# sanowl/CUDA-NT-Xent-MPI-NCCL-SimCLR

Hardware: AMD Instinct MI355X
Metric: NT-Xent fwd+bwd samples/sec, B=4096 d=2048, at 1/2/4/8 MI355X (higher is better)
Workload: dtype bf16

## Files before the change

cuda-nt-xent-mpi-nccl-simclr_amd/csrc/include/ntxent/ntxent.h:

```cpp
#pragma once

#include <hip/hip_runtime.h>

#include <cstdint>
#include <stdexcept>
#include <string>
#include <utility>
#include <vector>

namespace ntxent {

constexpr int kWaveSize = 64;
constexpr int kTile = 256;
constexpr int kTileElems = kTile * kTile;
constexpr int kKStepBytes = 128;
constexpr int kGemmThreads = 512;
constexpr int kLdsPerCU = 160 * 1024;
constexpr int kNumXcd = 8;

enum class DType : int { F32 = 0, F16 = 1, BF16 = 2, FP8 = 3 };

inline size_t dtype_size(DType t) { return t == DType::F32 ? 4 : (t == DType::FP8 ? 1 : 2); }
inline const char* dtype_name(DType t) {
  return t == DType::F32 ? "fp32" : (t == DType::F16 ? "fp16" : (t == DType::BF16 ? "bf16" : "fp8"));
// ... 130 lines not shown
void launch_lse(const float2* part, const float* ypos, float* lse2_all, float* cpos,
                float* block_loss, float* loss_sum, const Geometry& g, hipStream_t stream,
                DType tr_dtype = DType::F16, const void* zq = nullptr, void* zqt = nullptr,
                const Q8Stats* q8 = nullptr, const RawRows* raw = nullptr, bool fold_order = false);

int dot_slots(const Geometry& g);
void launch_coef(DType comp, const void* sbuf, void* cbuf, const float* lse2_all, const float* cpos,
                 const int4* tiles, int ntiles, const Geometry& g, hipStream_t stream,
                 void* mbuf = nullptr, float* dotp = nullptr, const Q8Stats* q8 = nullptr, bool half_c = false);
void launch_dot_reduce(const float* dotp, float* dot, const Geometry& g, hipStream_t stream);

void launch_coef_gemm(DType comp, const void* zq_local, const void* zq_all, void* cbuf,
                      const float* lse2_all, const float* cpos, const int4* tiles, int ntiles,
                      const GemmWorkspace& ws, const Geometry& g, hipStream_t stream,
                      const BlockView& bv = BlockView{}, float* dotp = nullptr);

struct NormFuse {
  const void* h = nullptr;
  DType in = DType::BF16;
  const float* inv = nullptr;
  const float* dot = nullptr;
  const float* grad_out = nullptr;
  void* dh = nullptr;
  const float* dotp = nullptr;
  int* dot_cnt = nullptr;
};
bool launch_dz(DType comp, const void* cbuf, const void* zqt_all, const int4* tiles, int ntiles,
               void* dz, const GemmWorkspace& ws, const Geometry& g, hipStream_t stream, bool out_f16 = false,
               const NormFuse* nf = nullptr, const Q8Stats* q8 = nullptr, const float* cpos = nullptr,
               bool half_c = false);
bool dz_half_c_eligible(DType comp, const Geometry& g, int n_dz, const GemmWorkspace& ws);
void set_half_c(bool on);
bool half_c_enabled();
bool dz_dot_fold_eligible(DType comp, const Geometry& g, int n_dz, const GemmWorkspace& ws);
void set_dot_fold(bool on);
bool dot_fold_enabled();
void set_dot_fold_spin(int polls);
int dot_fold_spin();

void launch_dz_view(DType comp, const void* a, long long a_panel_tiles, const void* b, long long b_kblk_cols,
                    long long b_kblk_stride, int k_tiles, const int4* tiles, int ntiles, void* out, bool accum,
                    const GemmWorkspace& ws, const Geometry& g, hipStream_t stream, bool out_f16 = false);

void launch_norm_bwd(DType in, const float* slabs, int nslabs, const void* h,
                     const float* inv, const float* grad_out, void* dh, const Geometry& g,
                     hipStream_t stream, const void* xslabs = nullptr, int nx = 0, float* dot_out = nullptr);

void launch_tau_grad(const float* dot, const float* grad_out, float* dtau, const Geometry& g, hipStream_t stream,
                     double* share64 = nullptr);

constexpr int kSmallMaxRows = 2048;
constexpr int kSmallMaxDk = 256;
bool small_path_eligible(const Geometry& g, DType comp);
int small_bwd_splits(const Geometry& g);
int small_rows_pad(const Geometry& g);
size_t small_scratch_bytes(const Geometry& g, int splits);
constexpr int kSmallFuseMaxRows = 1024;
bool small_fwd_fused(const Geometry& g);
void set_small_fuse_rows(int rows);
int small_fuse_rows_override();
void launch_small_fwd(DType in, DType comp, const void* h, void* zq, float* inv, float* ypos, float* lse2,
                      float* arow, float* loss, void* scratch, const Geometry& g, hipStream_t stream);
void launch_small_bwd(DType in, DType comp, const void* zq, const void* h, const float* inv, const float* lse2,
                      const float* arow, const float* grad_out, void* dh, void* scratch, const Geometry& g,
                      hipStream_t stream, int splits = 0, float* dot_out = nullptr);

// ... 56 lines not shown
```

cuda-nt-xent-mpi-nccl-simclr_amd/csrc/kernels/ntxent_kernels.hip:

```cpp

#include "../include/ntxent/ntxent.h"
#include "device_common.h"
#include "host_common.h"
#include "sim_gemm.h"

#include <atomic>
#include <algorithm>
#include <cmath>
#include <cstdio>
#include <cstdlib>
#include <mutex>
#include <string>
#include <type_traits>
#include <vector>
#include <unordered_map>

namespace ntxent {
namespace dev {

template <typename T> __device__ __forceinline__ void load8(const T* p, float (&v)[8]);
template <> __device__ __forceinline__ void load8<float>(const float* p, float (&v)[8]) {
  const f32x4 a = *reinterpret_cast<const f32x4*>(p), b = *reinterpret_cast<const f32x4*>(p + 4);
  v[0] = a[0]; v[1] = a[1]; v[2] = a[2]; v[3] = a[3]; v[4] = b[0]; v[5] = b[1]; v[6] = b[2]; v[7] = b[3];
}
// ... 722 lines not shown
  __syncthreads();
  if (threadIdx.x < 32 && blockIdx.x * 32 + (int)threadIdx.x < rows) {
    float t = 0.f;
#pragma unroll
    for (int g = 0; g < 8; ++g) t += part[g][threadIdx.x];
    dot[blockIdx.x * 32 + threadIdx.x] = t;
  }
}

constexpr int kTauGradThreads = 1024;
__global__ __launch_bounds__(kTauGradThreads) void tau_grad_kernel(const float* __restrict__ dot, int rows,
                                                                   const float* __restrict__ grad_out, double scale,
                                                                   float* __restrict__ dtau,
                                                                   double* __restrict__ share64) {
  __shared__ double part[kTauGradThreads];
  double t = 0.0;
  for (int i = threadIdx.x; i < rows; i += kTauGradThreads) t += (double)dot[i];
  part[threadIdx.x] = t;
  __syncthreads();
#pragma unroll
  for (int n = kTauGradThreads / 2; n > 0; n >>= 1) {
    if ((int)threadIdx.x < n) part[threadIdx.x] += part[threadIdx.x + n];
    __syncthreads();
  }
  if (threadIdx.x == 0) {
    const double v = (double)grad_out[0] * scale * part[0];
    if (dtau) dtau[0] = (float)v;
    else share64[0] = v;
  }
}

}

namespace {
void set_operand_scales(dev::SimParams& p, DType comp, const Geometry& g) {
  p.acc_scale = p.y_scale;
  p.scale_off = comp == DType::FP8 ? g.dim_k8 : 0;
}

#if NTXENT_TIMING
struct TimingBuf {
  unsigned long long* buf = nullptr;
  size_t cap = 0, n = 0;
  unsigned long long* prepare(int grid, hipStream_t stream) {
    n = (size_t)grid * dev::kTimingItems * dev::kTimingMarks;
    if (n > cap) {
      if (buf) NTXENT_HIP_CHECK(hipFree(buf));
      NTXENT_HIP_CHECK(hipMalloc(&buf, n * 8));
      cap = n;
    }
    NTXENT_HIP_CHECK(hipMemsetAsync(buf, 0, n * 8, stream));
    return buf;
  }
  void dump(const std::string& name, int grid, hipStream_t stream) const {
    const char* dir = std::getenv("NTXENT_TIMING_OUT");
    if (!dir) return;
    std::vector<unsigned long long> h(n);
    NTXENT_HIP_CHECK(hipStreamSynchronize(stream));
    NTXENT_HIP_CHECK(hipMemcpy(h.data(), buf, n * 8, hipMemcpyDeviceToHost));
    const std::string f = std::string(dir) + "/" + name + "_g" + std::to_string(grid) + ".bin";
    if (FILE* fp = std::fopen(f.c_str(), "wb")) {
      const int hdr[3] = {grid, dev::kTimingItems, dev::kTimingMarks};
      std::fwrite(hdr, sizeof(int), 3, fp);
      std::fwrite(h.data(), 8, n, fp);
      std::fclose(fp);
    }
  }
};
#endif

template <typename Tc, int MODE>
void launch_sim_gemm(int grid, const dev::SimParams& p_in, hipStream_t stream) {
#if NTXENT_TIMING
  static TimingBuf tb;
  dev::SimParams p = p_in;
  p.tstamp = tb.prepare(grid, stream);
#else
  const dev::SimParams& p = p_in;
#endif
  if (MODE == dev::kModeFwd && !p.fixed_shift)
    hipLaunchKernelGGL((dev::sim_gemm_kernel<Tc, MODE, MODE == dev::kModeFwd ? 0 : 1>), dim3(grid), dim3(kGemmThreads), 0,
                       stream, p);
  else
    hipLaunchKernelGGL((dev::sim_gemm_kernel<Tc, MODE>), dim3(grid), dim3(kGemmThreads), 0, stream, p);
#if NTXENT_TIMING
  tb.dump("gemm_m" + std::to_string(MODE) + "_e" + std::to_string(sizeof(Tc)), grid, stream);
#endif
}

dev::SimParams base_params(const Geometry& g) {
  dev::SimParams p{};
  p.R = g.rows;
  p.Rpad = g.rows_pad;
  p.n_half = g.rows / 2;
  p.own0 = g.rank * g.rows_pad;
  p.row_tile0 = g.rank * g.row_tiles;
  p.col_tiles = g.col_tiles;
  p.b_tile0 = 0;
  p.c_ld = g.col_tiles;
  p.c_tile0 = 0;
  p.y_scale = g.inv_temp * dev::kLog2e;
  p.acc_scale = p.y_scale;
  p.fixed_shift = (2.0f * p.y_scale < 120.0f) ? 1 : 0;
  return p;
}

constexpr int kDiagTickets = 14;
size_t sk_counter_bytes(int num_cus) {
  return ((size_t)std::max(2, kDiagTickets) * std::max(1, num_cus) * 4 + 255) / 256 * 256;
}

int apply_schedule(dev::SimParams& p, int ntiles, const GemmWorkspace& ws, hipStream_t stream) {
// ... 280 lines not shown
  });
  NTXENT_HIP_CHECK(hipGetLastError());
}

static std::atomic<bool> g_small_path{true};
static std::atomic<int> g_small_splits{0};
static std::atomic<int> g_small_fuse_rows{-1};
static std::atomic<bool> g_fp8_bwd{true};
static std::atomic<bool> g_raw_fwd{true};
void set_small_path(bool on) { g_small_path = on; }
bool small_path_enabled() { return g_small_path.load(); }
void set_small_splits(int n) { g_small_splits = std::max(0, n); }
int small_splits_override() { return g_small_splits.load(); }
void set_small_fuse_rows(int rows) { g_small_fuse_rows = rows < 0 ? -1 : rows; }
int small_fuse_rows_override() { return g_small_fuse_rows.load(); }
void set_fp8_backward(bool on) { g_fp8_bwd = on; }
void set_raw_forward(bool on) { g_raw_fwd = on; }

static std::atomic<bool> g_lse_fold{[] {
  const char* e = std::getenv("NTXENT_LSE_FOLD");
  return e == nullptr || std::string(e) != "0";
}()};
void set_lse_fold(bool on) { g_lse_fold = on; }

bool lse_fold_enabled() { return g_lse_fold.load(); }
static double lse_loss_fx(const Geometry& g, int nb);

static std::atomic<bool> g_half_c{[] {
  const char* e = std::getenv("NTXENT_HALF_C");
  return e == nullptr || std::string(e) != "0";
}()};
void set_half_c(bool on) { g_half_c = on; }
bool half_c_enabled() { return g_half_c.load(); }

bool dz_half_c_eligible(DType comp, const Geometry& g, int n_dz, const GemmWorkspace& ws) {
  if ((comp != DType::F16 && comp != DType::BF16) || g.world != 1 || n_dz <= 0) return false;
  if ((long long)g.row_tiles * g.col_tiles * kTileElems * 2 >= (1ll << 31)) return false;
  const int cus = ws.sched_cus > 0 ? std::min(ws.sched_cus, ws.num_cus) : ws.num_cus;
  const int nk = (int)((long long)g.rows_pad * 2 / kKStepBytes);
  int pieces = fwd_splitk_pieces(n_dz, nk, cus, 1);
  if (pieces < 3) pieces = 0;
  if (pieces > 0) return ((nk + pieces - 1) / pieces) % 2 == 0;
  return make_schedule(n_dz, nk, cus).sk_tiles == 0;
}
static std::atomic<bool> g_dot_fold{[] {
  const char* e = std::getenv("NTXENT_DOT_FOLD");
  return e == nullptr || std::string(e) != "0";
}()};
void set_dot_fold(bool on) { g_dot_fold = on; }
bool dot_fold_enabled() { return g_dot_fold.load(); }
static std::atomic<int> g_dot_spin{1 << 14};
void set_dot_fold_spin(int polls) { g_dot_spin = polls < 0 ? 0 : polls; }
int dot_fold_spin() { return g_dot_spin.load(); }
bool dz_dot_fold_eligible(DType comp, const Geometry& g, int n_dz, const GemmWorkspace&) {
  return (comp == DType::F16 || comp == DType::BF16) && n_dz > 0 && g.dim % 8 == 0 && dot_fold_enabled();
}
bool raw_forward_enabled() { return g_raw_fwd.load(); }
bool raw_forward_eligible(const Geometry& g, DType in, DType comp) {
  return g.world == 1 && (in == DType::F16 || in == DType::BF16) && (comp == DType::F16 || comp == in) &&
         g.rows % kTile == 0 && g.dim % 64 == 0 && g.dim <= 16384;
}
bool fp8_backward_enabled() { return g_fp8_bwd.load(); }
bool fp8_backward_eligible(const Geometry& g, DType comp) { return comp == DType::FP8 && g.world == 1 && g.dim % 8 == 0; }
int q8_ldt(const Geometry& g) { return (!NTXENT_NO_LDPAD && g.rows_pad % 1024 == 0) ? g.rows_pad + 128 : g.rows_pad; }

#ifndef NTXENT_ZT_SIDE_PER_CU
// ... 506 lines not shown
```

cuda-nt-xent-mpi-nccl-simclr_amd/csrc/kernels/sim_gemm.h:

```cpp
#pragma once

#include "../include/ntxent/ntxent.h"
#include "device_common.h"
#include "pair_mask.h"

#include <type_traits>

namespace ntxent {
namespace dev {

enum SimMode : int { kModeFwd = 0, kModeCoef = 1, kModeDz = 2 };

constexpr int kStageBytes = 2 * kTile * kKStepBytes;
#ifndef NTXENT_GEMM_DMA_AUX
#define NTXENT_GEMM_DMA_AUX 0
#endif
constexpr int kGemmDmaAux = NTXENT_GEMM_DMA_AUX;
#ifndef NTXENT_TIMING
#define NTXENT_TIMING 0
#endif
constexpr int kTimingItems = 8;
constexpr int kTimingMarks = 8;
__device__ __forceinline__ void store16_wt(void* base, long long off, u32x4 v) {
  const unsigned lo = __builtin_amdgcn_readfirstlane((unsigned)off);
  const unsigned hi = __builtin_amdgcn_readfirstlane((unsigned)((unsigned long long)off >> 32));
  const long long f0 = (long long)(((unsigned long long)hi << 32) | lo) - (64ll << 20);
  const long long wb = f0 > 0 ? (f0 & ~0xFFFFFll) : 0;
  const auto rs = __builtin_amdgcn_make_buffer_rsrc(static_cast<char*>(base) + wb, 0, 0x7FFFFFFF, 0x00020000);
  __builtin_amdgcn_raw_buffer_store_b128(v, rs, (int)(off - wb), 0, 16);
}

__device__ __forceinline__ long long ctile_off(int r, int c, int es) { return ((long long)r * kTile + c) * es; }
constexpr int kGemmLds = 2 * kStageBytes;
constexpr int kCtStride = kTile * 2 + 16;
constexpr int kCoefLds = kTile * kCtStride;
constexpr int kCoefWaveLds = 64 * (64 * 2 + 16);
constexpr int kHalfBytes = 128 * kKStepBytes;

struct OperandDesc {
  const char* base;
  long long row_tile_stride;
  long long ld;
  long long kblk;
  long long kblk_stride;
};

struct SimParams {
  OperandDesc A, B;
  const int4* tiles;
  long long kbytes;
  int R, Rpad, n_half, own0, row_tile0, col_tiles;
  int b_tile0;
  int c_ld, c_tile0;
  int c_rot;
  int c_half;
// ... 757 lines not shown
          op[1] = f32x4{o[4], o[5], o[6], o[7]};
        }
      }
      return;
    }
    _Float16* o16 = reinterpret_cast<_Float16*>(out) + ((long long)mt * kTile) * p.ldo + nt * kTile;
#pragma unroll 4
    for (int k = 0; k < 16; ++k) {
      const int idx = tid + kGemmThreads * k, rt = idx >> 5, c = idx & 31;
      const u32x4 v = *(lds_u4*)(lds + rt * 512 + ((c ^ (rt & 15)) << 4));
      *reinterpret_cast<u32x4*>(o16 + (long long)rt * p.ldo + c * 8) = v;
    }
  } else {
#pragma unroll
  for (int mi = 0; mi < 8; ++mi) {
    const long long row = (long long)mt * kTile + rb[mi] + (lane & 15);
#pragma unroll
    for (int ni = 0; ni < 4; ++ni) {
      const int col = nt * kTile + cb[ni] + 4 * (lane >> 4);
      if (p.out_f16) {
        union { _Float16 h[4]; u32x2 u; } pk;
#pragma unroll
        for (int r = 0; r < 4; ++r) pk.h[r] = (_Float16)acc[mi][ni][r];
        *reinterpret_cast<u32x2*>(reinterpret_cast<_Float16*>(out) + row * p.ldo + col) = pk.u;
      } else {
        f32x4* o = reinterpret_cast<f32x4*>(out + row * p.ldo + col);
        *o = p.accum ? *o + acc[mi][ni] : acc[mi][ni];
      }
    }
  }
  }
}

template <typename T, int MODE, int FX = 1>
__global__ __launch_bounds__(kGemmThreads) void sim_gemm_kernel(const SimParams p) {
  typedef typename Mfma<T>::frag frag;
  typedef __attribute__((address_space(3))) const frag lds_frag;
  constexpr int kScaleLds = MODE == kModeCoef ? kCoefLds : kGemmLds;
  constexpr int kFwdRed = kScaleLds + ((std::is_same<T, fp8e4m3>::value || MODE == kModeDz) ? 2048 : 0);
  constexpr int kInvLds = kFwdRed + (MODE == kModeFwd ? 6 * 256 * 8 : 0);
  __shared__ __attribute__((aligned(16))) char smem[kInvLds + (MODE == kModeFwd && !std::is_same<T, fp8e4m3>::value ? 4096 : 0) +
                                                     (MODE == kModeDz && !std::is_same<T, fp8e4m3>::value ? kHPieceExtra : 0)];
  lds_char* lds = (lds_char*)smem;
  typedef __attribute__((address_space(3))) u32x4 lds_u4;

  const int tid = threadIdx.x, lane = tid & 63, w = __builtin_amdgcn_readfirstlane(tid >> 6);
  const int wa = w >> 2, wb = w & 3;
  const int G = gridDim.x;
  const int bid = xcd_remap(blockIdx.x, G);
  const int nk = p.nk;
  KStream sa0, sa1, sb0, sb1;

  unsigned a_vo[2], b_vo[2];
#pragma unroll
  for (int j = 0; j < 2; ++j) {
    const int rl = 8 * j + (lane >> 3);
    const int lchunk = (lane & 7) ^ ((rl >> 1) & 7);
    a_vo[j] = (unsigned)((lane >> 3) * p.A.ld) + lchunk * 16;
    b_vo[j] = (unsigned)((lane >> 3) * p.B.ld) + lchunk * 16;
  }
  constexpr bool kTrCap = MODE == kModeDz && sizeof(T) == 2 && !std::is_same<T, fp8e4m3>::value;
  int tr_end = 0;
  const char* tr_base = nullptr;
  unsigned a_tr_vo = 0, rd_tr = 0;
  if constexpr (kTrCap) {
    const int x = w & 1;
    const int ch = 8 * (((lane >> 3) & 1) ^ x) + 2 * (lane >> 4) + (lane & 1);
// ... 89 lines not shown
        constexpr int sv = decltype(s_c)::value, mv = decltype(mi_c)::value;
        constexpr int off = OFF0 + 8 * sv * 1024 + 256 * mv;
        u32x2 lo, hi;
        asm volatile("ds_read_b64_tr_b16 %0, %2 offset:%c3\n\tds_read_b64_tr_b16 %1, %2 offset:%c4"
                     : "=&v"(lo), "=&v"(hi)
                     : "v"(base), "i"(off), "i"(off + 1024)
                     : "memory");
        af[sv][mv] = __builtin_bit_cast(OP, u32x4{lo[0], lo[1], hi[0], hi[1]});
      };
      typedef std::integral_constant<int, 0> J0;
      typedef std::integral_constant<int, 1> J1;
      typedef std::integral_constant<int, 2> J2;
      typedef std::integral_constant<int, 3> J3;
      one(J0{}, J0{}); one(J0{}, J1{}); one(J0{}, J2{}); one(J0{}, J3{});
      one(J1{}, J0{}); one(J1{}, J1{}); one(J1{}, J2{}); one(J1{}, J3{});
    }
  };
  auto read_b = [&](int buf, int h, OP (&bf)[NS][2]) {
    i32x4 lo[2];
#pragma unroll
    for (int s = 0; s < 2; ++s) {
#pragma unroll
      for (int ni = 0; ni < 2; ++ni) {
        const lds_char* src = lds + rd_b[s] + (buf * kTile + 128 * h + 16 * ni) * kKStepBytes;
        if constexpr (kF8) {
          if (s == 0) lo[ni] = *(lds_i4*)src;
          else bf[0][ni] = __builtin_shufflevector(lo[ni], *(lds_i4*)src, 0, 1, 2, 3, 4, 5, 6, 7);
        } else {
          bf[s][ni] = *(lds_frag*)src;
        }
      }
    }
  };
  auto mma_quadrant = [&](auto qa_c, auto qb_c, OP (&af)[NS][4], OP (&bf)[NS][2]) {
    constexpr int qa = decltype(qa_c)::value, qb = decltype(qb_c)::value;
    __builtin_amdgcn_s_setprio(1);
    if constexpr (kF8) {
      auto mx = [&](auto mi_c, auto ni_c) {
        constexpr int mi = decltype(mi_c)::value, ni = decltype(ni_c)::value;
        f32x4& c = acc[qa * 4 + mi][qb * 2 + ni];
        if constexpr (MODE == kModeDz)
          c = mma_mx_c<qb * 2 + ni, mi>(bf[0][ni], af[0][mi], c, kUnitScale, kUnitScale);
        else
          c = mma_mx_c<mi, qb * 2 + ni>(af[0][mi], bf[0][ni], c, sa_v[qa], sb_v);
        asm volatile("" ::"v"(c));
      };
      typedef std::integral_constant<int, 0> I0;
      typedef std::integral_constant<int, 1> I1;
      typedef std::integral_constant<int, 2> I2;
      typedef std::integral_constant<int, 3> I3;
      mx(I0{}, I0{}); mx(I0{}, I1{}); mx(I1{}, I0{}); mx(I1{}, I1{});
      mx(I2{}, I0{}); mx(I2{}, I1{}); mx(I3{}, I0{}); mx(I3{}, I1{});
    } else {
#pragma unroll
      for (int s = 0; s < 2; ++s)
#pragma unroll
        for (int mi = 0; mi < 4; ++mi)
#pragma unroll
          for (int ni = 0; ni < 2; ++ni) {
            f32x4& c = acc[qa * 4 + mi][qb * 2 + ni];
            c = MODE == kModeDz ? Mfma<T>::mma(bf[s][ni], af[s][mi], c) : Mfma<T>::mma(af[s][mi], bf[s][ni], c);
          }
    }
    __builtin_amdgcn_s_setprio(0);
  };
  const std::integral_constant<int, 0> kI0{};
  const std::integral_constant<int, 1> kI1{};
  auto barrier = [&]() {
    __builtin_amdgcn_s_barrier();
    asm volatile("" ::: "memory");
  };
  auto lds_drain = [&]() { asm volatile("s_waitcnt lgkmcnt(0)" ::: "memory"); };
  auto a0_retire = [&]() { asm volatile("s_waitcnt lgkmcnt(4)" ::: "memory"); };
  constexpr bool kStreamMode = MODE == kModeFwd && !kF8;
  auto dma_wait = [&]() { asm volatile("s_waitcnt vmcnt(8)" ::: "memory"); };
  const int grp = __builtin_amdgcn_readfirstlane(w) >> 2;

  const long long sk_total = (long long)p.sk_tiles * nk;
  const long long it0 = (long long)bid * p.ipb;
  const long long it1 = it0 + p.ipb < sk_total ? it0 + p.ipb : sk_total;
  const int n_dp = p.dp_tiles > bid ? (p.dp_tiles - bid + G - 1) / G : 0;
  long long it = it0;
  auto fetch = [&](int item, int& tile, int& kb, int& ke, int& stile) -> bool {
    stile = -1;
    if (item < n_dp) {
      tile = bid + item * G;
      kb = 0;
      ke = nk;
      return true;
    }
    if (p.splitk) {
      if (item > 0) return false;
      stile = bid % p.sk_tiles;
      kb = (int)((bid / p.sk_tiles) * p.ipb);
      ke = kb + (int)p.ipb < nk ? kb + (int)p.ipb : nk;
      tile = p.dp_tiles + stile;
      return true;
    }
    if (it >= it1) return false;
    stile = (int)(it / nk);
    kb = (int)(it % nk);
    ke = (int)((long long)kb + (it1 - it) < nk ? kb + (it1 - it) : nk);
    it += ke - kb;
    tile = p.dp_tiles + stile;
    return true;
  };
  auto prologue = [&](int tile, int kb, int ke, int slot) {
    const int4 tt = sload_int4(p.tiles, tile);
    if (p.inv_a) stage_inv(tt.x, tt.y, slot);
    if constexpr (kTrCap) {
// ... 3 lines not shown
    const int ns = ke - kb;
    const char* Ab = p.A.base + (long long)tt.x * p.A.row_tile_stride;
    const char* Bb = p.B.base + (long long)(tt.y - p.b_tile0) * p.B.row_tile_stride;
    const long long k0 = (long long)kb * kKStepBytes;
    sa0.init(Ab, k0, p.A, ns); sa1.init(Ab, k0, p.A, ns);
    if constexpr (kTrCap) {
      if (tr_end > kb) {
        sa0.seek(Ab, (long long)tr_end * kKStepBytes, p.A);
        sa1.seek(Ab, (long long)tr_end * kKStepBytes, p.A);
      }
    }
    sb0.init(Bb, k0, p.B, ns); sb1.init(Bb, k0, p.B, ns);
    if constexpr (kF8 && MODE != kModeDz) {
      const int t = threadIdx.x;
      const char* src = (t < 256 ? Ab + (long long)t * p.A.ld : Bb + (long long)(t - 256) * p.B.ld) + p.scale_off;
      __builtin_amdgcn_global_load_lds((const void*)src, (lds_void*)(lds + kScaleLds + 256 * w), 4, 0, 0);
    }
    stage(0, 0, sa0, 0); stage(1, 0, sb0, 0); stage(1, 1, sb1, 0); stage(0, 1, sa1, 0);
    stage(0, 0, sa0, 1); stage(1, 0, sb0, 1); stage(1, 1, sb1, 1);
  };
  const bool streaming = kStreamMode && p.sk_tiles == 0 && nk >= 2 && (nk & 1) == 0;
  bool streamed = false;
  int dstate = 0;
  bool dot_counted = false;
  if constexpr (MODE == kModeDz && !kF8 && sizeof(T) == 2) {
    if (p.dot_nslot > 0) dz_dot_fold(p, lds + kGemmLds, threadIdx.x);
  }
  auto tmark = [&](int item, int k) {
#if NTXENT_TIMING
    if (threadIdx.x == 0 && item < kTimingItems)
      p.tstamp[((long long)blockIdx.x * kTimingItems + item) * kTimingMarks + k] = __builtin_amdgcn_s_memtime();
#endif
  };
  for (int item = 0;; ++item) {
  tmark(item, 0);
  int tile, kb, ke, stile;
  if (streamed) {
    tile = bid + item * G; kb = 0; ke = nk; stile = -1;
  } else {
    if (!fetch(item, tile, kb, ke, stile)) break;
    prologue(tile, kb, ke, item & 1);
  }
  const bool cont = streaming && item + 1 < n_dp;
  const char* na = nullptr;
  const char* nb = nullptr;
  int nmt = 0, nnt = 0;
  if (cont) {
    const int4 tn = sload_int4(p.tiles, bid + (item + 1) * G);
    na = p.A.base + (long long)tn.x * p.A.row_tile_stride;
    nb = p.B.base + (long long)(tn.y - p.b_tile0) * p.B.row_tile_stride;
    nmt = tn.x;
    nnt = tn.y;
  }
  const int4 t = sload_int4(p.tiles, tile);
  const int mt = t.x, nt = t.y;
  const int nsteps = ke - kb;
#pragma unroll
  for (int mi = 0; mi < 8; ++mi)
#pragma unroll
    for (int ni = 0; ni < 4; ++ni) acc[mi][ni] = f32x4{0.f, 0.f, 0.f, 0.f};

  asm volatile("s_waitcnt vmcnt(10)" ::: "memory");
  barrier();
  if constexpr (MODE == kModeDz && !kF8 && sizeof(T) == 2) {
    if (item == 0 && p.dot_cnt != nullptr && threadIdx.x == 0)
      __hip_atomic_fetch_add(p.dot_cnt, 1, __ATOMIC_RELAXED, __HIP_MEMORY_SCOPE_AGENT);
    dot_counted = true;
  }
  if constexpr (kF8 && MODE != kModeDz) {
    const int r16_ = lane & 15;
    unsigned av[8], bv[4];
    lds_get_scales((unsigned)(uintptr_t)(lds + kScaleLds) + 4 * (64 * wa + r16_),
                   (unsigned)(uintptr_t)(lds + kScaleLds) + 4 * (256 + 32 * wb + r16_), av, bv);
    sa_v[0] = pack_low_bytes(av[0], av[1], av[2], av[3]);
    sa_v[1] = pack_low_bytes(av[4], av[5], av[6], av[7]);
    sb_v = pack_low_bytes(bv[0], bv[1], bv[2], bv[3]);
  }
  tmark(item, 1);
  if (grp == 1) barrier();
  bool hpre = false;
  if constexpr (MODE == kModeDz && !kF8)
    hpre = p.ndh != nullptr && (p.nh_dt == 1 || p.nh_dt == 2) && stile < 0 && nsteps == nk && nsteps >= 4 &&
           (nsteps & 1) == 0 && p.R % kTile == 0 && p.nd % kTile == 0;
  auto kstep = [&](const int ks, auto cur_c, auto tail_c, auto tr_c) {
    constexpr int cur = decltype(cur_c)::value, nxt = cur ^ 1;
    constexpr int TAIL = decltype(tail_c)::value;
    constexpr bool TR = decltype(tr_c)::value != 0;
    constexpr int TRM = decltype(tr_c)::value == 0 ? 0 : (decltype(tr_c)::value == 2 ? 1 : 2);
    if constexpr (kStreamMode) {
      if (cont && ks == nsteps - 2) {
        sa0.init(na, 0, p.A, nk); sb0.init(nb, 0, p.B, nk); sb1.init(nb, 0, p.B, nk);
        if (p.inv_a) stage_inv(nmt, nnt, (item + 1) & 1);
      }
      if (cont && ks == nsteps - 1) sa1.init(na, 0, p.A, nk);
    }
    dma_wait(); barrier();
    if constexpr (TR) read_a_tr(cur_c, kI0, af);
    else read_a(cur, 0, af);
    __builtin_amdgcn_sched_barrier(0);
    read_b(cur, 0, bf0);
    if constexpr (TAIL == 2) stage_h(3, mt, nt);
    else stage(0, 1, sa1, nxt, TRM);
    a0_retire(); barrier();
    lds_drain();
    if constexpr (TR) __builtin_amdgcn_sched_barrier(0);
    mma_quadrant(kI0, kI0, af, bf0);
    dma_wait(); barrier();
    read_b(cur, 1, bf1);
    if constexpr (TAIL != 0) stage_h(TAIL == 1 ? 0 : 4, mt, nt);
    else stage(0, 0, sa0, cur, TRM);
    barrier(); lds_drain();
    mma_quadrant(kI0, kI1, af, bf1);
    barrier();
    if constexpr (TR) read_a_tr(cur_c, kI1, af);
    else read_a(cur, 1, af);
    if constexpr (TAIL != 0) stage_h(TAIL == 1 ? 1 : 5, mt, nt);
    else stage(1, 0, sb0, cur);
    barrier(); lds_drain();
    if constexpr (TR) __builtin_amdgcn_sched_barrier(0);
    mma_quadrant(kI1, kI0, af, bf0);
    if constexpr (TAIL != 2) dma_wait();
    barrier();
    if constexpr (TAIL != 0) {
      stage_h(TAIL == 1 ? 2 : 6, mt, nt);
      if constexpr (TAIL == 2) stage_h(7, mt, nt);
    } else {
      stage(1, 1, sb1, cur);
    }
    barrier();
    mma_quadrant(kI1, kI1, af, bf1);
  };
  const std::integral_constant<int, 2> kI2{};
  int ks2 = 0;
  const int nmain = nsteps - (hpre ? 2 : 0);
  if constexpr (kTrCap) {
    const int ntr = tr_end > kb ? (tr_end < ke ? tr_end : ke) - kb : 0;
    for (; ks2 + 3 < ntr; ks2 += 2) {
      kstep(ks2, kI0, kI0, kI1);
      kstep(ks2 + 1, kI1, kI0, kI1);
    }
    if (ks2 + 1 < ntr) {
      kstep(ks2, kI0, kI0, kI2);
      kstep(ks2 + 1, kI1, kI0, kI2);
      ks2 += 2;
    }
  }
  for (; ks2 + 1 < nmain; ks2 += 2) {
    kstep(ks2, kI0, kI0, kI0);
    kstep(ks2 + 1, kI1, kI0, kI0);
  }
  if constexpr (MODE == kModeDz && !kF8) {
    if (hpre) {
      kstep(ks2, kI0, kI1, kI0);
      kstep(ks2 + 1, kI1, kI2, kI0);
      ks2 += 2;
    }
  }
  if (ks2 < nsteps) kstep(ks2, kI0, kI0, kI0);
  if (grp == 0) barrier();
  tmark(item, 2);
  float hiv = 0.f, hdt = 0.f;
  if constexpr (MODE == kModeDz && !kF8) {
    if (hpre && threadIdx.x < kTile) {
      hiv = p.ninv[mt * kTile + threadIdx.x];
      hdt = dz_dot<sizeof(T) == 2>(p, mt * kTile + threadIdx.x, dstate);
    }
  }
  if (kStreamMode && cont) {
    streamed = true;
  } else {
    streamed = false;
    asm volatile("s_waitcnt vmcnt(0)" ::: "memory");
  }
  if constexpr (kStreamMode) {
    lds_drain();
    barrier();
  } else {
    __syncthreads();
  }
  {
  int tid_e = threadIdx.x;
  asm volatile("" : "+v"(tid_e));
  const int tid = tid_e, lane = tid_e & 63, w = tid_e >> 6;
  const int wa = w >> 2, wb = w & 3;
  int rb[8], cb[4];
#pragma unroll
  for (int mi = 0; mi < 8; ++mi) rb[mi] = 128 * (mi >> 2) + 64 * wa + 16 * (mi & 3);
#pragma unroll
  for (int ni = 0; ni < 4; ++ni) cb[ni] = 128 * (ni >> 1) + 32 * wb + 16 * (ni & 1);

  if constexpr (MODE == kModeFwd && !kF8) {
    if (p.inv_a) {
      const unsigned ib = (unsigned)(uintptr_t)(lds + kInvLds) + (unsigned)((item & 1) * 2048);
// ... 836 lines not shown
```

cuda-nt-xent-mpi-nccl-simclr_amd/csrc/runtime/ntxent_torch.cpp:

```cpp
#include <torch/extension.h>
#include <ATen/hip/impl/HIPGuardImplMasqueradingAsCUDA.h>
#include <ATen/hip/impl/HIPStreamMasqueradingAsCUDA.h>
#include <ATen/hip/impl/HIPCachingAllocatorMasqueradingAsCUDA.h>

#include <algorithm>
#include <map>
#include <memory>
#include <atomic>
#include <mutex>
#include <string>
#include <tuple>
#include <vector>

#include "ntxent/engine.h"
#include "ntxent/ntxent.h"
#include "ntxent/step.h"
#include "ntxent/sym_step.h"
#include "../kernels/pair_mask.h"

namespace ntxent {
namespace th {

DType to_dtype(at::ScalarType t) {
  switch (t) {
// ... 1334 lines not shown
  m.def("rccl_unique_id", []() { return py::bytes(ntxent::RcclComm::unique_id()); });
  m.def("get_plan", &get_plan, py::arg("rows"), py::arg("dim"), py::arg("world"), py::arg("rank"),
        py::arg("temperature"), py::arg("compute"), py::arg("device"));
  m.def("choose_compute", [](const std::string& in_dtype, bool mp, const std::string& ov) {
    at::ScalarType t = in_dtype == "float32" ? at::kFloat : (in_dtype == "float16" ? at::kHalf : at::kBFloat16);
    return std::string(ntxent::dtype_name(choose_compute(t, mp, ov)));
  });
  m.def("prep", &prep, py::arg("h"), py::arg("plan"), py::arg("zq_out") = py::none(), py::arg("zq8_out") = py::none());
  m.def("transpose", &transpose, py::arg("zq"), py::arg("plan"), py::arg("zqt_out") = py::none());
  m.def("pos_rank", &pos_rank, py::arg("zq"), py::arg("plan"),
        "Stage op: (rank, pos_cos, hard_neg_cos) of prep's unit rows zq for a world-1 plan.");
  m.def("positive_rank", &positive_rank, py::arg("h"), py::arg("compute") = "auto",
        py::arg("use_mixed_precision") = false,
        "(rank, pos_cos, hard_neg_cos) of stacked views h = [h1; h2] on the current stream: rank[i] counts the "
        "negatives whose cosine is strictly larger than the positive's. compute: auto|fp32|fp16|bf16|fp8, "
        "resolved as for the loss; fp8 computes in fp16.");
  m.def("fwd_stats_range", &fwd_stats_range, py::arg("zq_local"), py::arg("zq_all"), py::arg("plan"), py::arg("part"),
        py::arg("sc"), py::arg("first"), py::arg("count"), py::arg("reserve_cus") = 0);
  m.def("fwd_stats", [](const at::Tensor& zl, const at::Tensor& za, const Plan& P, bool keep) {
    return fwd_stats(zl, za, P, keep, true);
  }, py::arg("zq_local"), py::arg("zq_all"), py::arg("plan"), py::arg("keep_cos"));
  m.def("lse", &lse, py::arg("part"), py::arg("ypos"), py::arg("lse2_all"), py::arg("cpos"), py::arg("plan"),
        py::arg("zq") = py::none(), py::arg("zqt") = py::none());
  m.def("coef", &coef, py::arg("sbuf"), py::arg("lse2_all"), py::arg("cpos"), py::arg("plan"));
  m.def("coef_gemm", &coef_gemm);
  m.def("dz", &dz);
  m.def("set_fp8_backward", &ntxent::set_fp8_backward, py::arg("on"));
  m.def("set_raw_forward", &ntxent::set_raw_forward, py::arg("on"));
  m.def("raw_forward_enabled", &ntxent::raw_forward_enabled);
  m.def("set_lse_fold", &ntxent::set_lse_fold, py::arg("on"));
  m.def("lse_fold_enabled", &ntxent::lse_fold_enabled);
  m.def("set_half_c", &ntxent::set_half_c, py::arg("on"));
  m.def("half_c_enabled", &ntxent::half_c_enabled);
  m.def("set_dot_fold", &ntxent::set_dot_fold, py::arg("on"));
  m.def("dot_fold_enabled", &ntxent::dot_fold_enabled);
  m.def("set_dot_fold_spin", &ntxent::set_dot_fold_spin, py::arg("polls"));
  m.def("dot_fold_spin", &ntxent::dot_fold_spin);
  m.def("fp8_backward_enabled", &ntxent::fp8_backward_enabled);
  m.def("fwd_splitk_pieces", &ntxent::fwd_splitk_pieces, py::arg("ntiles"), py::arg("nk"), py::arg("cus"),
        py::arg("diag_tail"));
  m.def("fwd_diag_remainder", &ntxent::fwd_diag_remainder, py::arg("ntiles"), py::arg("nk"), py::arg("cus"),
        py::arg("diag_tail"), py::arg("f8") = false);
  m.def("norm_bwd", &norm_bwd, py::arg("slabs"), py::arg("h"), py::arg("inv"), py::arg("grad_out"), py::arg("plan"));
  m.def("fwd_stats_tiles", &fwd_stats_tiles, py::arg("zq_local"), py::arg("zq_chunk"), py::arg("b_tile0"),
        py::arg("tiles"), py::arg("plan"), py::arg("part"), py::arg("reserve_cus") = 0);
  m.def("coef_gemm_tiles", &coef_gemm_tiles, py::arg("zq_local"), py::arg("zq_chunk"), py::arg("b_tile0"),
        py::arg("tiles"), py::arg("lse2_all"), py::arg("cpos"), py::arg("plan"), py::arg("c_ld"), py::arg("c_tile0"),
        py::arg("reserve_cus") = 0);
  m.def("dz_block", &dz_block, py::arg("cbuf_block"), py::arg("zqt_chunk"), py::arg("plan"), py::arg("reserve_cus") = 0);
  m.def("dz_view", &dz_view, py::arg("abuf"), py::arg("a_tile0"), py::arg("a_panel_tiles"), py::arg("bbuf"),
        py::arg("b_block0"), py::arg("b_col0"), py::arg("k_tiles"), py::arg("m0"), py::arg("m1"), py::arg("out"),
        py::arg("accum"), py::arg("plan"), py::arg("reserve_cus") = 0);
  {
    const auto plan = py::arg("plan"), bufs = py::arg("bufs");
    const auto reserve = py::arg("reserve_cus") = 0;
    py::class_<SymStep, std::shared_ptr<SymStep>>(m, "SymStep")
        .def_property_readonly("plan", [](const SymStep& S) { return sym_plan_dict(S.sp); })
        .def("prep", sym_phase<>([](const SymStep& S, const Plan& P, SymBundle& x, hipStream_t s) {
          ntxent::sym_prep(S.sp, P.g, x.in, x.b, s);
        }), plan, bufs)
        .def("fwd_tiles_range", sym_phase<int, int, int>([](const SymStep& S, const Plan& P, SymBundle& x, hipStream_t s,
                                                            int first, int count, int reserve_cus) {
          ntxent::sym_fwd_tiles(S.sp, P.g, P.comp, x.b, first, count, gemm_ws(x.like, count, P, reserve_cus), s);
        }), plan, bufs, py::arg("first"), py::arg("count"), reserve)
        .def("lse", sym_phase<>([](const SymStep& S, const Plan& P, SymBundle& x, hipStream_t s) {
          x.b.block_loss = static_cast<float*>(device_scratch(x.like, (size_t)ntxent::lse_scratch_floats(P.g) * 4, 1).data_ptr());
// ... 149 lines not shown
```

Measured before the change: 11.21 million.

## Add two-phase k-step schedule for bf16/fp16 dz GEMM, on by default

Adds a SCHED=2 variant of the similarity GEMM k-step that splits each step into two phases. Each phase reads an A half and both B fragments, then issues two MFMA quadrants back to back, which halves the barriers and DMA waits per step compared with the four-quadrant schedule. The variant is on by default for the dz backward GEMM (fp16/bf16, no split-k) and can be toggled per mode through an env var or Python setters. It also adds finer timing marks and a compile-time switch that disables MFMA for profiling. Holding more fragments live may raise register pressure, and the new vmcnt wait counts must match the DMA issue order.

```diff
diff --git a/cuda-nt-xent-mpi-nccl-simclr_amd/csrc/include/ntxent/ntxent.h b/cuda-nt-xent-mpi-nccl-simclr_amd/csrc/include/ntxent/ntxent.h
--- a/cuda-nt-xent-mpi-nccl-simclr_amd/csrc/include/ntxent/ntxent.h
+++ b/cuda-nt-xent-mpi-nccl-simclr_amd/csrc/include/ntxent/ntxent.h
@@ -186,6 +186,9 @@
 bool dz_half_c_eligible(DType comp, const Geometry& g, int n_dz, const GemmWorkspace& ws);
 void set_half_c(bool on);
 bool half_c_enabled();
+void set_gemm_two_phase(bool on, int which = -1);
+bool gemm_two_phase_enabled(bool dz);
+long long gemm_two_phase_launches(bool dz);
 bool dz_dot_fold_eligible(DType comp, const Geometry& g, int n_dz, const GemmWorkspace& ws);
 void set_dot_fold(bool on);
 bool dot_fold_enabled();
diff --git a/cuda-nt-xent-mpi-nccl-simclr_amd/csrc/kernels/ntxent_kernels.hip b/cuda-nt-xent-mpi-nccl-simclr_amd/csrc/kernels/ntxent_kernels.hip
--- a/cuda-nt-xent-mpi-nccl-simclr_amd/csrc/kernels/ntxent_kernels.hip
+++ b/cuda-nt-xent-mpi-nccl-simclr_amd/csrc/kernels/ntxent_kernels.hip
@@ -778,6 +778,8 @@
 
 }
 
+static void count_two_phase_launch(bool dz);
+
 namespace {
 void set_operand_scales(dev::SimParams& p, DType comp, const Geometry& g) {
   p.acc_scale = p.y_scale;
@@ -824,6 +826,22 @@
 #else
   const dev::SimParams& p = p_in;
 #endif
+  constexpr bool kTwoCap = !std::is_same<Tc, float>::value && !std::is_same<Tc, dev::fp8e4m3>::value &&
+                           (MODE == dev::kModeFwd || MODE == dev::kModeDz);
+  if constexpr (kTwoCap) {
+    if (gemm_two_phase_enabled(MODE == dev::kModeDz) && p.sk_tiles == 0 && !p.splitk) {
+      count_two_phase_launch(MODE == dev::kModeDz);
+      if (MODE == dev::kModeFwd && !p.fixed_shift)
+        hipLaunchKernelGGL((dev::sim_gemm_kernel<Tc, MODE, MODE == dev::kModeFwd ? 0 : 1, 2>), dim3(grid),
+                           dim3(kGemmThreads), 0, stream, p);
+      else
+        hipLaunchKernelGGL((dev::sim_gemm_kernel<Tc, MODE, 1, 2>), dim3(grid), dim3(kGemmThreads), 0, stream, p);
+#if NTXENT_TIMING
+      tb.dump("gemm_m" + std::to_string(MODE) + "_e" + std::to_string(sizeof(Tc)), grid, stream);
+#endif
+      return;
+    }
+  }
   if (MODE == dev::kModeFwd && !p.fixed_shift)
     hipLaunchKernelGGL((dev::sim_gemm_kernel<Tc, MODE, MODE == dev::kModeFwd ? 0 : 1>), dim3(grid), dim3(kGemmThreads), 0,
                        stream, p);
@@ -1170,6 +1188,24 @@
 }()};
 void set_half_c(bool on) { g_half_c = on; }
 bool half_c_enabled() { return g_half_c.load(); }
+
+static constexpr bool kTwoPhaseDefault[2] = {false, true};
+static std::atomic<bool> g_two_phase[2];
+static const bool g_two_phase_init = [] {
+  const char* e = std::getenv("NTXENT_TWO_PHASE");
+  const std::string v = e ? e : "";
+  g_two_phase[0] = e == nullptr ? kTwoPhaseDefault[0] : (v == "fwd" || (v != "0" && v != "dz"));
+  g_two_phase[1] = e == nullptr ? kTwoPhaseDefault[1] : (v == "dz" || (v != "0" && v != "fwd"));
+  return true;
+}();
+void set_gemm_two_phase(bool on, int which) {
+  if (which != 1) g_two_phase[0] = on;
+  if (which != 0) g_two_phase[1] = on;
+}
+bool gemm_two_phase_enabled(bool dz) { return g_two_phase[dz ? 1 : 0].load(); }
+static std::atomic<long long> g_two_phase_launches[2];
+static void count_two_phase_launch(bool dz) { ++g_two_phase_launches[dz ? 1 : 0]; }
+long long gemm_two_phase_launches(bool dz) { return g_two_phase_launches[dz ? 1 : 0].load(); }
 
 bool dz_half_c_eligible(DType comp, const Geometry& g, int n_dz, const GemmWorkspace& ws) {
   if ((comp != DType::F16 && comp != DType::BF16) || g.world != 1 || n_dz <= 0) return false;
diff --git a/cuda-nt-xent-mpi-nccl-simclr_amd/csrc/kernels/sim_gemm.h b/cuda-nt-xent-mpi-nccl-simclr_amd/csrc/kernels/sim_gemm.h
--- a/cuda-nt-xent-mpi-nccl-simclr_amd/csrc/kernels/sim_gemm.h
+++ b/cuda-nt-xent-mpi-nccl-simclr_amd/csrc/kernels/sim_gemm.h
@@ -20,7 +20,10 @@
 #define NTXENT_TIMING 0
 #endif
 constexpr int kTimingItems = 8;
-constexpr int kTimingMarks = 8;
+constexpr int kTimingMarks = 32;
+#ifndef NTXENT_NO_MFMA
+#define NTXENT_NO_MFMA 0
+#endif
 __device__ __forceinline__ void store16_wt(void* base, long long off, u32x4 v) {
   const unsigned lo = __builtin_amdgcn_readfirstlane((unsigned)off);
   const unsigned hi = __builtin_amdgcn_readfirstlane((unsigned)((unsigned long long)off >> 32));
@@ -844,7 +847,7 @@
   }
 }
 
-template <typename T, int MODE, int FX = 1>
+template <typename T, int MODE, int FX = 1, int SCHED = 4>
 __global__ __launch_bounds__(kGemmThreads) void sim_gemm_kernel(const SimParams p) {
   typedef typename Mfma<T>::frag frag;
   typedef __attribute__((address_space(3))) const frag lds_frag;
@@ -1000,10 +1003,17 @@
       }
     }
   };
-  auto mma_quadrant = [&](auto qa_c, auto qb_c, OP (&af)[NS][4], OP (&bf)[NS][2]) {
+  auto mma_quadrant_raw = [&](auto qa_c, auto qb_c, OP (&af)[NS][4], OP (&bf)[NS][2]) __attribute__((always_inline)) {
     constexpr int qa = decltype(qa_c)::value, qb = decltype(qb_c)::value;
-    __builtin_amdgcn_s_setprio(1);
-    if constexpr (kF8) {
+    if constexpr (NTXENT_NO_MFMA != 0 && !kF8) {
+#pragma unroll
+      for (int s = 0; s < NS; ++s) {
+#pragma unroll
+        for (int mi = 0; mi < 4; ++mi) asm volatile("" ::"v"(af[s][mi]));
+#pragma unroll
+        for (int ni = 0; ni < 2; ++ni) asm volatile("" ::"v"(bf[s][ni]));
+      }
+    } else if constexpr (kF8) {
       auto mx = [&](auto mi_c, auto ni_c) {
         constexpr int mi = decltype(mi_c)::value, ni = decltype(ni_c)::value;
         f32x4& c = acc[qa * 4 + mi][qb * 2 + ni];
@@ -1030,6 +1040,16 @@
             c = MODE == kModeDz ? Mfma<T>::mma(bf[s][ni], af[s][mi], c) : Mfma<T>::mma(af[s][mi], bf[s][ni], c);
           }
     }
+  };
+  auto mma_quadrant = [&](auto qa_c, auto qb_c, OP (&af)[NS][4], OP (&bf)[NS][2]) __attribute__((always_inline)) {
+    __builtin_amdgcn_s_setprio(1);
+    mma_quadrant_raw(qa_c, qb_c, af, bf);
+    __builtin_amdgcn_s_setprio(0);
+  };
+  auto mma_half = [&](auto qa_c, OP (&af)[NS][4], OP (&bf0)[NS][2], OP (&bf1)[NS][2]) __attribute__((always_inline)) {
+    __builtin_amdgcn_s_setprio(1);
+    mma_quadrant_raw(qa_c, std::integral_constant<int, 0>{}, af, bf0);
+    mma_quadrant_raw(qa_c, std::integral_constant<int, 1>{}, af, bf1);
     __builtin_amdgcn_s_setprio(0);
   };
   const std::integral_constant<int, 0> kI0{};
@@ -1044,6 +1064,8 @@
   auto dma_wait = [&]() { asm volatile("s_waitcnt vmcnt(8)" ::: "memory"); };
   const int grp = __builtin_amdgcn_readfirstlane(w) >> 2;
 
+  auto dma_wait_a = [&]() { asm volatile("s_waitcnt vmcnt(6)" ::: "memory"); };
+  auto dma_wait_b = [&]() { asm volatile("s_waitcnt vmcnt(2)" ::: "memory"); };
   const long long sk_total = (long long)p.sk_tiles * nk;
   const long long it0 = (long long)bid * p.ipb;
   const long long it1 = it0 + p.ipb < sk_total ? it0 + p.ipb : sk_total;
@@ -1113,6 +1135,25 @@
       p.tstamp[((long long)blockIdx.x * kTimingItems + item) * kTimingMarks + k] = __builtin_amdgcn_s_memtime();
 #endif
   };
+#if NTXENT_TIMING
+  unsigned tks[17];
+  int tmid = -8;
+  auto kmark = [&](int ks, auto cur_c, auto b_c) {
+    constexpr int cur = decltype(cur_c)::value, b = decltype(b_c)::value;
+    auto now = [&]() {
+      unsigned long long t;
+      asm volatile("s_memtime %0\n\ts_waitcnt lgkmcnt(0)" : "=s"(t)::"memory");
+      return (unsigned)t;
+    };
+    if (ks == tmid + cur) tks[8 * cur + b] = now();
+    if constexpr (cur == 0 && b == 0) {
+      if (ks == tmid + 2) tks[16] = now();
+    }
+  };
+#define NTXENT_KMARK(B) kmark(ks, cur_c, std::integral_constant<int, B>{})
+#else
+#define NTXENT_KMARK(B)
+#endif
   for (int item = 0;; ++item) {
   tmark(item, 0);
   int tile, kb, ke, stile;
@@ -1141,7 +1182,9 @@
 #pragma unroll
     for (int ni = 0; ni < 4; ++ni) acc[mi][ni] = f32x4{0.f, 0.f, 0.f, 0.f};
 
-  asm volatile("s_waitcnt vmcnt(10)" ::: "memory");
+  constexpr bool two = SCHED == 2;
+  if constexpr (two) asm volatile("s_waitcnt vmcnt(8)" ::: "memory");
+  else asm volatile("s_waitcnt vmcnt(10)" ::: "memory");
   barrier();
   if constexpr (MODE == kModeDz && !kF8 && sizeof(T) == 2) {
     if (item == 0 && p.dot_cnt != nullptr && threadIdx.x == 0)
@@ -1163,7 +1206,13 @@
   if constexpr (MODE == kModeDz && !kF8)
     hpre = p.ndh != nullptr && (p.nh_dt == 1 || p.nh_dt == 2) && stile < 0 && nsteps == nk && nsteps >= 4 &&
            (nsteps & 1) == 0 && p.R % kTile == 0 && p.nd % kTile == 0;
-  auto kstep = [&](const int ks, auto cur_c, auto tail_c, auto tr_c) {
+  const std::integral_constant<int, 2> kI2{};
+  const std::integral_constant<int, 3> kI3{};
+  const std::integral_constant<int, 4> kI4{};
+  const std::integral_constant<int, 5> kI5{};
+  const std::integral_constant<int, 6> kI6{};
+  const std::integral_constant<int, 7> kI7{};
+  auto kstep2 = [&](const int ks, auto cur_c, auto tail_c, auto tr_c) __attribute__((always_inline)) {
     constexpr int cur = decltype(cur_c)::value, nxt = cur ^ 1;
     constexpr int TAIL = decltype(tail_c)::value;
     constexpr bool TR = decltype(tr_c)::value != 0;
@@ -1175,7 +1224,53 @@
       }
       if (cont && ks == nsteps - 1) sa1.init(na, 0, p.A, nk);
     }
+    dma_wait_a(); barrier();
+    NTXENT_KMARK(0);
+    if constexpr (TR) read_a_tr(cur_c, kI0, af);
+    else read_a(cur, 0, af);
+    read_b(cur, 0, bf0);
+    read_b(cur, 1, bf1);
+    if constexpr (TAIL == 2) stage_h(3, mt, nt);
+    else stage(0, 1, sa1, nxt, TRM);
+    lds_drain(); barrier();
+    NTXENT_KMARK(1);
+    if constexpr (TR) __builtin_amdgcn_sched_barrier(0);
+    mma_half(kI0, af, bf0, bf1);
+    if constexpr (TAIL != 2) dma_wait_b();
+    barrier();
+    NTXENT_KMARK(2);
+    if constexpr (TR) read_a_tr(cur_c, kI1, af);
+    else read_a(cur, 1, af);
+    if constexpr (TAIL == 1) {
+      stage_h(0, mt, nt); stage_h(1, mt, nt); stage_h(2, mt, nt);
+    } else if constexpr (TAIL == 2) {
+      stage_h(4, mt, nt); stage_h(5, mt, nt); stage_h(6, mt, nt);
+      stage_h(7, mt, nt);
+    } else {
+      stage(0, 0, sa0, cur, TRM);
+      stage(1, 0, sb0, cur);
+      stage(1, 1, sb1, cur);
+    }
+    lds_drain(); barrier();
+    NTXENT_KMARK(3);
+    if constexpr (TR) __builtin_amdgcn_sched_barrier(0);
+    mma_half(kI1, af, bf0, bf1);
+  };
+  auto kstep = [&](const int ks, auto cur_c, auto tail_c, auto tr_c) {
+    if constexpr (two) return kstep2(ks, cur_c, tail_c, tr_c);
+    constexpr int cur = decltype(cur_c)::value, nxt = cur ^ 1;
+    constexpr int TAIL = decltype(tail_c)::value;
+    constexpr bool TR = decltype(tr_c)::value != 0;
+    constexpr int TRM = decltype(tr_c)::value == 0 ? 0 : (decltype(tr_c)::value == 2 ? 1 : 2);
+    if constexpr (kStreamMode) {
+      if (cont && ks == nsteps - 2) {
+        sa0.init(na, 0, p.A, nk); sb0.init(nb, 0, p.B, nk); sb1.init(nb, 0, p.B, nk);
+        if (p.inv_a) stage_inv(nmt, nnt, (item + 1) & 1);
+      }
+      if (cont && ks == nsteps - 1) sa1.init(na, 0, p.A, nk);
+    }
     dma_wait(); barrier();
+    NTXENT_KMARK(0);
     if constexpr (TR) read_a_tr(cur_c, kI0, af);
     else read_a(cur, 0, af);
     __builtin_amdgcn_sched_barrier(0);
@@ -1183,25 +1278,33 @@
     if constexpr (TAIL == 2) stage_h(3, mt, nt);
     else stage(0, 1, sa1, nxt, TRM);
     a0_retire(); barrier();
+    NTXENT_KMARK(1);
     lds_drain();
     if constexpr (TR) __builtin_amdgcn_sched_barrier(0);
     mma_quadrant(kI0, kI0, af, bf0);
     dma_wait(); barrier();
+    NTXENT_KMARK(2);
     read_b(cur, 1, bf1);
     if constexpr (TAIL != 0) stage_h(TAIL == 1 ? 0 : 4, mt, nt);
     else stage(0, 0, sa0, cur, TRM);
-    barrier(); lds_drain();
+    barrier();
+    NTXENT_KMARK(3);
+    lds_drain();
     mma_quadrant(kI0, kI1, af, bf1);
     barrier();
+    NTXENT_KMARK(4);
     if constexpr (TR) read_a_tr(cur_c, kI1, af);
     else read_a(cur, 1, af);
     if constexpr (TAIL != 0) stage_h(TAIL == 1 ? 1 : 5, mt, nt);
     else stage(1, 0, sb0, cur);
-    barrier(); lds_drain();
+    barrier();
+    NTXENT_KMARK(5);
+    lds_drain();
     if constexpr (TR) __builtin_amdgcn_sched_barrier(0);
     mma_quadrant(kI1, kI0, af, bf0);
     if constexpr (TAIL != 2) dma_wait();
     barrier();
+    NTXENT_KMARK(6);
     if constexpr (TAIL != 0) {
       stage_h(TAIL == 1 ? 2 : 6, mt, nt);
       if constexpr (TAIL == 2) stage_h(7, mt, nt);
@@ -1209,9 +1312,14 @@
       stage(1, 1, sb1, cur);
     }
     barrier();
+    NTXENT_KMARK(7);
     mma_quadrant(kI1, kI1, af, bf1);
   };
-  const std::integral_constant<int, 2> kI2{};
+#if NTXENT_TIMING
+  tmid = nsteps >= 8 ? (nsteps / 2) & ~1 : -8;
+#pragma unroll
+  for (int i = 0; i < 17; ++i) tks[i] = 0;
+#endif
   int ks2 = 0;
   const int nmain = nsteps - (hpre ? 2 : 0);
   if constexpr (kTrCap) {
@@ -1240,6 +1348,16 @@
   if (ks2 < nsteps) kstep(ks2, kI0, kI0, kI0);
   if (grp == 0) barrier();
   tmark(item, 2);
+#if NTXENT_TIMING
+  if (threadIdx.x == 0 && item < kTimingItems) {
+    unsigned long long* ts = p.tstamp + ((long long)blockIdx.x * kTimingItems + item) * kTimingMarks;
+#pragma unroll
+    for (int i = 0; i < 17; ++i) ts[8 + i] = tks[i];
+    ts[25] = (unsigned long long)(tmid > 0 ? tmid : 0);
+    ts[26] = (unsigned long long)tr_end;
+    ts[27] = two ? 1 : 0;
+  }
+#endif
   float hiv = 0.f, hdt = 0.f;
   if constexpr (MODE == kModeDz && !kF8) {
     if (hpre && threadIdx.x < kTile) {
diff --git a/cuda-nt-xent-mpi-nccl-simclr_amd/csrc/runtime/ntxent_torch.cpp b/cuda-nt-xent-mpi-nccl-simclr_amd/csrc/runtime/ntxent_torch.cpp
--- a/cuda-nt-xent-mpi-nccl-simclr_amd/csrc/runtime/ntxent_torch.cpp
+++ b/cuda-nt-xent-mpi-nccl-simclr_amd/csrc/runtime/ntxent_torch.cpp
@@ -1390,6 +1390,9 @@
   m.def("lse_fold_enabled", &ntxent::lse_fold_enabled);
   m.def("set_half_c", &ntxent::set_half_c, py::arg("on"));
   m.def("half_c_enabled", &ntxent::half_c_enabled);
+  m.def("set_gemm_two_phase", &ntxent::set_gemm_two_phase, py::arg("on"), py::arg("which") = -1);
+  m.def("gemm_two_phase_enabled", &ntxent::gemm_two_phase_enabled, py::arg("dz"));
+  m.def("gemm_two_phase_launches", &ntxent::gemm_two_phase_launches, py::arg("dz"));
   m.def("set_dot_fold", &ntxent::set_dot_fold, py::arg("on"));
   m.def("dot_fold_enabled", &ntxent::dot_fold_enabled);
   m.def("set_dot_fold_spin", &ntxent::set_dot_fold_spin, py::arg("polls"));
```

Result: no change. 11.32 million, median of 6 (+1.0%).
